# rlorenzo/facet

Measured on AMD Instinct MI355X. Metric: images/sec whole-node (TOPIQ+SAMP+CLIP+InsightFace ensemble), 1024² batch, higher is better.
Workload: dtype f32

## Files before the change

facet_amd/csrc/engine.hip:

```cpp
#include "engine.h"
#include "onnx_graph.h"
#include "wino64_maps.h"
#include <algorithm>
#include <cmath>
#include <cstdlib>

namespace fe {

void WeightStore::set(const std::string& name, const float* data, const int64_t* shape, int ndim) {
  HostTensor h;
  h.shape.assign(shape, shape + ndim);
  h.data.assign(data, data + h.numel());
  t_[name] = std::move(h);
}
const HostTensor& WeightStore::get(const std::string& name) const {
  auto it = t_.find(name);
  if (it == t_.end()) throw Error("missing weight tensor '" + name + "'");
  return it->second;
}

float* DeviceWeights::upload(const std::vector<float>& v) {
  void* p = nullptr;
  const size_t b = v.size() * sizeof(float);
  FE_HIP(hipMalloc(&p, b ? b : 16));
// ... 213 lines not shown

void conv_forward(Ctx& c, const ConvW& w, const Tensor& x, const Tensor& y, const ConvOpts& o) {
  FE_CHECK(x.c == w.CinPad, "conv: input channels %d != packed Cin %d", x.c, w.CinPad);
  FE_CHECK(y.c == w.Cout && y.n == x.n, "conv: output view mismatch (c=%d Cout=%d)", y.c, w.Cout);
  ConvParams p{};
  p.x = x.p; p.ldx = x.ld;
  p.w = w.w; p.scale = w.scale; p.shift = w.shift; p.slope = w.slope;
  FE_CHECK(o.act != ACT_PRELU || w.slope, "conv: PReLU without slopes");
  if (o.res) {
    FE_CHECK(o.res->c == y.c && o.res->pixels() == y.pixels(), "conv: residual shape mismatch");
    p.res = o.res->p; p.ldr = o.res->ld;
  }
  if (o.gate) {
    FE_CHECK(o.gate->pixels() == y.pixels() && (o.gate->c == 1 || o.gate->c == y.c), "conv: gate shape mismatch");
    p.gate = o.gate->p; p.ldg = o.gate->ld; p.gate_c1 = o.gate->c == 1;
  }
  p.y = y.p; p.ldy = y.ld;
  p.N = x.n; p.H = x.h; p.W = x.w; p.Cin = w.CinPad;
  p.Ho = y.h; p.Wo = y.w; p.Cout = w.Cout;
  p.KH = w.KH; p.KW = w.KW; p.sh = o.sh; p.sw = o.sw; p.ph = o.ph; p.pw = o.pw; p.dh = o.dh; p.dw = o.dw;
  FE_CHECK(y.h == conv_out_dim(x.h, w.KH, o.sh, o.ph, o.dh) && y.w == conv_out_dim(x.w, w.KW, o.sw, o.pw, o.dw),
           "conv: output dims %dx%d inconsistent with input %dx%d", y.h, y.w, x.h, x.w);
  p.K = w.K; p.Kp = w.Kp;
  p.M = (int)y.pixels();
  FE_CHECK(y.pixels() < (1ull << 31), "conv: M too large");
  p.act = o.act; p.res_after_act = o.res_after_act;
  p.variant = c.force_variant;
  if (w.wtap && o.act != ACT_PRELU && o.sh == 1 && o.sw == 1 && !o.res && !o.gate && p.variant == 0 && y.h == x.h && y.w == x.w) {
    const int T = w.KH * w.KW * w.Cout, Tp = (T + 3) & ~3;
    const size_t mark = c.arena.mark();
    Tensor z = c.arena.tensor(x.n, x.h, x.w, Tp);
    ConvParams q{};
    q.x = x.p; q.ldx = x.ld; q.w = w.wtap; q.y = z.p; q.ldy = Tp;
    q.N = x.n; q.H = x.h; q.W = x.w; q.Cin = w.CinPad; q.Ho = x.h; q.Wo = x.w; q.Cout = T;
    q.KH = q.KW = 1; q.sh = q.sw = q.dh = q.dw = 1;
    q.K = w.CinPad; q.Kp = w.KpT; q.M = (int)x.pixels();
    launch_conv(q, c.stream);
    launch_tap_gather(z.p, Tp, x.n, x.h, x.w, w.KH, w.KW, o.ph, o.pw, o.dh, o.dw, w.Cout, w.scale, w.shift, o.act, y.p,
                      y.ld, y.h, y.w, c.stream);
    c.arena.rewind(mark);
    c.flops_accum += 2.0 * p.M * (double)(w.KH * w.KW * w.Cin) * (w.CoutAlg ? w.CoutAlg : p.Cout);
    return;
  }
  static const bool no_wino = getenv("FE_NO_WINO") != nullptr;
  const bool wino_plain = !o.res && (o.act == ACT_NONE || o.act == ACT_RELU);
  if (w.wino && !no_wino && p.variant == 0 && o.sh == 1 && o.sw == 1 && o.ph == 1 && o.pw == 1 && o.dh == 1 && o.dw == 1 &&
      !o.gate && (wino_plain || (w.wino_m == 4 && (o.act == ACT_NONE || o.act == ACT_RELU || o.act == ACT_PRELU))) && y.h == x.h && y.w == x.w && (((uintptr_t)x.p | (uintptr_t)y.p) & 15) == 0 &&
      x.ld % 4 == 0 && y.ld % 4 == 0) {
    const int ts = w.wino_m, planes = (ts + 2) * (ts + 2);
    const int th = (x.h + ts - 1) / ts, tw = (x.w + ts - 1) / ts;
    const size_t tiles = (size_t)x.n * th * tw;
    const size_t wino_bytes = (size_t)planes * tiles * ((size_t)w.CinPad + w.Cout) * sizeof(float) + 1024;
    if (tiles < (1u << 30) / 36 && c.arena.mark() + wino_bytes <= c.arena.capacity()) {
      const size_t mark = c.arena.mark();
      float* V = (float*)c.arena.alloc((size_t)planes * tiles * w.CinPad * sizeof(float));
      float* Mb = (float*)c.arena.alloc((size_t)planes * tiles * w.Cout * sizeof(float));
      hipEvent_t e0 = nullptr, e1 = nullptr;
      if (c.profile) {
        FE_HIP(hipEventCreate(&e0)); FE_HIP(hipEventCreate(&e1));
        FE_HIP(hipEventRecord(e0, c.stream));
      }
      if (ts == 2) launch_wino_input(x, th, tw, V, c.stream);
      else launch_wino4_input(x, th, tw, V, c.stream);
      ConvParams g{};
      g.x = V; g.ldx = w.CinPad; g.w = w.wino; g.ldw = w.CinPad; g.y = Mb; g.ldy = w.Cout;
      g.M = (int)tiles; g.K = w.CinPad; g.Cout = w.Cout;
      g.N = 1; g.H = 1; g.W = g.M; g.Ho = 1; g.Wo = g.M; g.KH = g.KW = 1; g.sh = g.sw = g.dh = g.dw = 1;
      g.Kp = w.CinPad; g.Cin = w.CinPad;
      g.batch = planes; g.nb1 = 1; g.xs2 = (long long)tiles * w.CinPad; g.ws2 = (long long)w.Cout * w.CinPad; g.ys2 = (long long)tiles * w.Cout;
      launch_conv(g, c.stream);
      if (ts == 2) launch_wino_output(Mb, y, th, tw, w.scale, w.shift, o.act == ACT_RELU, c.stream);
      else launch_wino4_output(Mb, y, th, tw, w.scale, w.shift, o.act, w.slope, o.res, o.res_after_act, c.stream);
      if (c.profile) {
        FE_HIP(hipEventRecord(e1, c.stream));
        FE_HIP(hipEventSynchronize(e1));
        float ms = 0.f;
        FE_HIP(hipEventElapsedTime(&ms, e0, e1));
        (void)hipEventDestroy(e0); (void)hipEventDestroy(e1);
        char nm[128];
        snprintf(nm, sizeof nm, "wino3x3 M=%d K=%d N=%d", p.M, p.K, p.Cout);
        c.timings.push_back({nm, 2.0 * p.M * (double)(9 * w.Cin) * p.Cout, 0.0, ms});
      }
      c.arena.rewind(mark);
      c.flops_accum += 2.0 * p.M * (double)(w.KH * w.KW * w.Cin) * (w.CoutAlg ? w.CoutAlg : p.Cout);
      c.flops_saved += 2.0 * p.M * (double)(9 * w.Cin) * (w.CoutAlg ? w.CoutAlg : p.Cout) - 2.0 * (double)planes * (double)tiles * w.CinPad * w.Cout;
      return;
    }
  }
  static const bool no_wino64 = getenv("FE_NO_WINO64") != nullptr;
  if (w.wino64 && !no_wino64 && p.variant == 0 && (o.act == ACT_NONE || o.act == ACT_RELU || o.act == ACT_PRELU) && o.sh == 1 && o.sw == 1 && o.ph == 1 && o.pw == 1 && o.dh == 1 && o.dw == 1 && !o.gate && y.h == x.h &&
      y.w == x.w && (((uintptr_t)x.p | (uintptr_t)y.p | (uintptr_t)(o.res ? o.res->p : nullptr)) & 15) == 0 && x.ld % 4 == 0 && y.ld % 4 == 0 &&
      (!o.res || o.res->ld % 4 == 0) && (unsigned long long)x.h * x.w * x.ld * 4ull < 0xF0000000ull) {
    hipEvent_t e0 = nullptr, e1 = nullptr;
    if (c.profile) {
      FE_HIP(hipEventCreate(&e0)); FE_HIP(hipEventCreate(&e1));
      FE_HIP(hipEventRecord(e0, c.stream));
    }
    launch_wino64(x, y, w.wino64, w.scale, w.shift, w.slope, o.act, o.res, o.res_after_act, c.stream);
    const double direct = 2.0 * p.M * (double)(9 * w.Cin) * (w.CoutAlg ? w.CoutAlg : p.Cout);
    if (c.profile) {
      FE_HIP(hipEventRecord(e1, c.stream));
      FE_HIP(hipEventSynchronize(e1));
      float ms = 0.f;
      FE_HIP(hipEventElapsedTime(&ms, e0, e1));
      (void)hipEventDestroy(e0); (void)hipEventDestroy(e1);
      char nm[128];
      snprintf(nm, sizeof nm, "wino64 3x3 M=%d K=%d N=%d", p.M, p.K, p.Cout);
      const double bytes = 4.0 * ((double)x.pixels() * x.c + (double)y.pixels() * y.c * (o.res ? 2 : 1) + (double)w64::U_FLOATS);
      c.timings.push_back({nm, direct, bytes, ms});
    }
    const double tiles = (double)x.n * ((x.h + 1) / 2) * ((x.w + 1) / 2);
    c.flops_accum += direct;
    c.flops_saved += direct - 2.0 * 16.0 * tiles * 64.0 * w.Cout;
    return;
  }
  static const bool no_splitk = getenv("FE_NO_SPLITK") != nullptr;
  static const int splitk_min = getenv("FE_SPLITK_MIN") ? atoi(getenv("FE_SPLITK_MIN")) : 2048;
  if (!no_splitk && w.KH == 1 && w.KW == 1 && o.sh == 1 && o.sw == 1 && o.ph == 0 && o.pw == 0 && !o.gate && p.variant == 0 && p.M <= 256 &&
      w.CinPad >= splitk_min && w.K == w.CinPad && (size_t)((p.M + 127) / 128) * ((w.Cout + 63) / 64) < 64 &&
      (o.act == ACT_NONE || o.act == ACT_RELU || o.act == ACT_PRELU)) {
    int splits = 0;
    for (int s = 64; s >= 2; --s)
      if (w.CinPad % s == 0 && (w.CinPad / s) % 32 == 0 && w.CinPad / s >= 256) { splits = s; break; }
    const size_t part_bytes = (size_t)splits * p.M * w.Cout * sizeof(float);
    if (splits && c.arena.mark() + part_bytes + 1024 <= c.arena.capacity()) {
      const size_t mark = c.arena.mark();
      float* part = (float*)c.arena.alloc(part_bytes);
      const int Ks = w.CinPad / splits;
      hipEvent_t e0 = nullptr, e1 = nullptr;
      if (c.profile) {
        FE_HIP(hipEventCreate(&e0)); FE_HIP(hipEventCreate(&e1));
        FE_HIP(hipEventRecord(e0, c.stream));
      }
      ConvParams g{};
      g.x = x.p; g.ldx = x.ld; g.w = w.w; g.ldw = w.Kp; g.y = part; g.ldy = w.Cout;
      g.M = p.M; g.K = Ks; g.Kp = Ks; g.Cin = Ks; g.Cout = w.Cout;
      g.N = 1; g.H = 1; g.W = g.M; g.Ho = 1; g.Wo = g.M; g.KH = g.KW = 1; g.sh = g.sw = g.dh = g.dw = 1;
      g.batch = splits; g.nb1 = 1; g.xs2 = Ks; g.ws2 = Ks; g.ys2 = (long long)p.M * w.Cout;
      launch_conv(g, c.stream);
      launch_splitk_reduce(part, splits, p.M, w.Cout, w.scale, w.shift, w.slope, o.act, o.res ? o.res->p : nullptr, o.res ? o.res->ld : 0,
                           o.res_after_act, y.p, y.ld, c.stream);
      if (c.profile) {
        FE_HIP(hipEventRecord(e1, c.stream));
        FE_HIP(hipEventSynchronize(e1));
        float ms = 0.f;
        FE_HIP(hipEventElapsedTime(&ms, e0, e1));
        (void)hipEventDestroy(e0); (void)hipEventDestroy(e1);
        char nm[128];
        snprintf(nm, sizeof nm, "splitk%d 1x1 M=%d K=%d N=%d", splits, p.M, p.K, p.Cout);
        c.timings.push_back({nm, 2.0 * p.M * (double)w.Cin * (w.CoutAlg ? w.CoutAlg : p.Cout), 0.0, ms});
      }
      c.arena.rewind(mark);
      c.flops_accum += 2.0 * p.M * (double)w.Cin * (w.CoutAlg ? w.CoutAlg : p.Cout);
      return;
    }
  }
  static const bool no_stem = getenv("FE_NO_STEM") != nullptr;
  const bool stem = w.wstem && !no_stem && p.variant == 0 && o.sh == o.sw && o.ph == w.KH / 2 && o.pw == w.KW / 2 && o.dh == 1 && o.dw == 1 && !o.res &&
                    !o.gate && (o.act == ACT_NONE || o.act == ACT_RELU || o.act == ACT_PRELU);
  auto launch = [&]() {
    if (stem && launch_stem(x.p, x.ld, x.n, x.h, x.w, w.wstem, w.scale, w.shift, w.slope, w.Cout, w.KH, o.sh,
                            o.act == ACT_RELU ? 1 : (o.act == ACT_PRELU ? 2 : 0), y.p, y.ld, y.h, y.w, c.stream))
      return;
    launch_conv(p, c.stream);
  };
  if (c.profile) {
    hipEvent_t e0, e1;
    FE_HIP(hipEventCreate(&e0)); FE_HIP(hipEventCreate(&e1));
    FE_HIP(hipEventRecord(e0, c.stream));
    launch();
    FE_HIP(hipEventRecord(e1, c.stream));
    FE_HIP(hipEventSynchronize(e1));
    float ms = 0.f;
    FE_HIP(hipEventElapsedTime(&ms, e0, e1));
    (void)hipEventDestroy(e0); (void)hipEventDestroy(e1);
    char nm[128];
    snprintf(nm, sizeof nm, "conv%dx%d s%d d%d M=%d K=%d N=%d", w.KH, w.KW, o.sh, o.dh, p.M, p.K, p.Cout);
    double bytes = 4.0 * ((double)x.pixels() * x.c + (double)y.pixels() * y.c * (o.res ? 2 : 1) + (double)w.Cout * w.K);
    c.timings.push_back({nm, 2.0 * p.M * (double)(w.KH * w.KW * w.Cin) * (w.CoutAlg ? w.CoutAlg : p.Cout), bytes, ms});
  } else {
    launch();
  }
  c.flops_accum += 2.0 * p.M * (double)(w.KH * w.KW * w.Cin) * (w.CoutAlg ? w.CoutAlg : p.Cout);
}

template <class E>
static void conv_forward_half(Ctx& c, const ConvW& w, const TensorT<E>& x, const TensorT<E>& y, const ConvOptsT<E>& o) {
  if (!w.wh && w.w && PrecOf<E>::value != PREC_F32 && !o.res && !o.gate && x.ld == x.c && y.ld == y.c && x.c >= w.CinPad) {
    const size_t mark = c.arena.mark();
    Tensor xf = c.arena.tensor(x.n, x.h, x.w, x.c), yf = c.arena.tensor(y.n, y.h, y.w, y.c);
    launch_convert(x.p, xf.p, x.numel(), c.stream);
    ConvOpts of; of.sh = o.sh; of.sw = o.sw; of.ph = o.ph; of.pw = o.pw; of.dh = o.dh; of.dw = o.dw; of.act = o.act;
    conv_forward(c, w, xf.slice(0, w.CinPad), yf, of);
    launch_convert(yf.p, y.p, y.numel(), c.stream);
    c.arena.rewind(mark);
    return;
  }
  FE_CHECK(w.wh && w.hprec == PrecOf<E>::value, "conv(2-byte): this layer has no weights of the activations' type (model committed under another "
           "precision, or a 3-channel first layer)");
  FE_CHECK(x.c == w.CinPadH, "conv(bf16): input channels %d != packed Cin %d", x.c, w.CinPadH);
  FE_CHECK(y.c == w.Cout && y.n == x.n, "conv(bf16): output view mismatch (c=%d Cout=%d)", y.c, w.Cout);
  FE_CHECK(y.p || o.y32, "conv(2-byte): no output tensor");
  FE_CHECK(y.h == conv_out_dim(x.h, w.KH, o.sh, o.ph, o.dh) && y.w == conv_out_dim(x.w, w.KW, o.sw, o.pw, o.dw),
           "conv(bf16): output dims %dx%d inconsistent with input %dx%d", y.h, y.w, x.h, x.w);
  FE_CHECK(y.pixels() < (1ull << 31), "conv: M too large");
  const double flops = 2.0 * (double)y.pixels() * (double)(w.KH * w.KW * w.Cin) * (w.CoutAlg ? w.CoutAlg : w.Cout);
  hipEvent_t e0 = nullptr, e1 = nullptr;
  if (c.profile) {
    FE_HIP(hipEventCreate(&e0)); FE_HIP(hipEventCreate(&e1));
    FE_HIP(hipEventRecord(e0, c.stream));
  }
  ConvParamsT<E> p{};
  p.scale = w.scale; p.shift = w.shift; p.slope = w.slope;
  p.N = x.n; p.H = x.h; p.W = x.w; p.Cin = w.CinPadH; p.x = x.p; p.ldx = x.ld;
  if (w.wtap_h && o.act != ACT_PRELU && o.sh == 1 && o.sw == 1 && !o.res && !o.gate && !o.res32 && !o.y32 && y.h == x.h && y.w == x.w) {
    const int T = w.KH * w.KW * w.Cout, T8 = (T + 7) & ~7;
    const size_t mark = c.arena.mark();
    TensorT<E> z = c.arena.tensor_t<E>(x.n, x.h, x.w, T8);
    p.w = (const E*)w.wtap_h; p.y = z.p; p.ldy = T8; p.scale = p.shift = p.slope = nullptr;
    p.Ho = x.h; p.Wo = x.w; p.Cout = T8; p.KH = p.KW = 1; p.sh = p.sw = p.dh = p.dw = 1;
    p.K = w.CinPadH; p.Kp = w.KpTH; p.M = (int)x.pixels(); p.cb = 32;
    launch_conv_bf16(p, c.stream);
    launch_tap_gather(z.p, T8, x.n, x.h, x.w, w.KH, w.KW, o.ph, o.pw, o.dh, o.dw, w.Cout, w.scale, w.shift, o.act, y.p, y.ld, y.h, y.w, c.stream);
    c.arena.rewind(mark);
  } else {
    FE_CHECK(o.act != ACT_PRELU || w.slope, "conv: PReLU without slopes");
    if (o.res) {
      FE_CHECK(o.res->c == y.c && o.res->pixels() == y.pixels(), "conv: residual shape mismatch");
      p.res = o.res->p; p.ldr = o.res->ld;
    }
    if (o.gate) {
      FE_CHECK(o.gate->pixels() == y.pixels() && (o.gate->c == 1 || o.gate->c == y.c), "conv: gate shape mismatch");
      p.gate = o.gate->p; p.ldg = o.gate->ld; p.gate_c1 = o.gate->c == 1;
    }
    if (o.res32) {
      FE_CHECK(!o.res && o.res32->c == y.c && o.res32->pixels() == y.pixels(), "conv: fp32 residual shape mismatch");
      p.res32 = o.res32->p; p.ldr32 = o.res32->ld;
    }
    if (o.y32) {
      FE_CHECK(o.y32->c == y.c && o.y32->pixels() == y.pixels(), "conv: fp32 output shape mismatch");
      p.y32 = o.y32->p; p.ldy32 = o.y32->ld;
    }
    p.w = (const E*)w.wh; p.y = y.p; p.ldy = y.ld;
    p.Ho = y.h; p.Wo = y.w; p.Cout = w.Cout;
    p.KH = w.KH; p.KW = w.KW; p.sh = o.sh; p.sw = o.sw; p.ph = o.ph; p.pw = o.pw; p.dh = o.dh; p.dw = o.dw;
    p.K = w.KH * w.KW * w.CinPadH; p.Kp = w.KpH; p.M = (int)y.pixels(); p.cb = w.cb;
    p.act = o.act; p.res_after_act = o.res_after_act;
    p.variant = c.force_variant;
    launch_conv_bf16(p, c.stream);
  }
  if (c.profile) {
    FE_HIP(hipEventRecord(e1, c.stream));
    FE_HIP(hipEventSynchronize(e1));
    float ms = 0.f;
    FE_HIP(hipEventElapsedTime(&ms, e0, e1));
    (void)hipEventDestroy(e0); (void)hipEventDestroy(e1);
    char nm[128];
    snprintf(nm, sizeof nm, "%s conv%dx%d s%d d%d M=%d K=%d N=%d", PrecOf<E>::value == PREC_F16 ? "f16" : "bf16", w.KH, w.KW, o.sh, o.dh, (int)y.pixels(), w.KH * w.KW * w.Cin, w.Cout);
    const double bytes = 2.0 * ((double)x.pixels() * x.c + (double)y.pixels() * y.c * (o.res ? 2 : 1) + (double)w.Cout * w.KpH);
    c.timings.push_back({nm, flops, bytes, ms});
  }
  c.flops_accum += flops;
  c.flops_half += flops;
}
void conv_forward(Ctx& c, const ConvW& w, const TensorH& x, const TensorH& y, const ConvOptsT<bf16>& o) { conv_forward_half<bf16>(c, w, x, y, o); }
void conv_forward(Ctx& c, const ConvW& w, const TensorF16& x, const TensorF16& y, const ConvOptsT<f16>& o) { conv_forward_half<f16>(c, w, x, y, o); }

template <class T>
TensorT<T> conv_new(Ctx& c, const ConvW& w, const TensorT<T>& x, const ConvOptsT<T>& o) {
  TensorT<T> y = c.arena.tensor_t<T>(x.n, conv_out_dim(x.h, w.KH, o.sh, o.ph, o.dh), conv_out_dim(x.w, w.KW, o.sw, o.pw, o.dw), w.Cout);
  conv_forward(c, w, x, y, o);
  return y;
}
template Tensor conv_new<float>(Ctx&, const ConvW&, const Tensor&, const ConvOpts&);
template TensorH conv_new<bf16>(Ctx&, const ConvW&, const TensorH&, const ConvOptsT<bf16>&);
template TensorF16 conv_new<f16>(Ctx&, const ConvW&, const TensorF16&, const ConvOptsT<f16>&);

template <>
Tensor first_conv<float>(Ctx& c, const ConvW& w, const Tensor& x, const ConvOpts& o) { return conv_new(c, w, x, o); }
template <class E>
static TensorT<E> first_conv_half(Ctx& c, const ConvW& w, const Tensor& x, const ConvOpts& o) {
  const int ho = conv_out_dim(x.h, w.KH, o.sh, o.ph, o.dh), wo = conv_out_dim(x.w, w.KW, o.sw, o.pw, o.dw);
  TensorT<E> y = c.arena.tensor_t<E>(x.n, ho, wo, w.Cout);
  static const bool no_stem = getenv("FE_NO_STEM") != nullptr;
  const bool stem = w.wstem && !no_stem && o.sh == o.sw && o.ph == w.KH / 2 && o.pw == w.KW / 2 && o.dh == 1 && o.dw == 1 && !o.res && !o.gate &&
                    (o.act == ACT_NONE || o.act == ACT_RELU || o.act == ACT_PRELU);
  if (stem && launch_stem(x.p, x.ld, x.n, x.h, x.w, w.wstem, w.scale, w.shift, w.slope, w.Cout, w.KH, o.sh,
                          o.act == ACT_RELU ? 1 : (o.act == ACT_PRELU ? 2 : 0), y.p, y.ld, ho, wo, c.stream)) {
    c.flops_accum += 2.0 * (double)y.pixels() * (double)(w.KH * w.KW * w.Cin) * w.Cout;
    if (w.KH == 7) c.flops_half += 2.0 * (double)y.pixels() * (double)(w.KH * w.KW * w.Cin) * w.Cout;
    return y;
  }
  const size_t mark = c.arena.mark();
  Tensor yf = conv_new(c, w, x, o);
  launch_convert(yf.p, y.p, y.numel(), c.stream);
  (void)mark;
  return y;
}
template <>
TensorH first_conv<bf16>(Ctx& c, const ConvW& w, const Tensor& x, const ConvOpts& o) { return first_conv_half<bf16>(c, w, x, o); }
template <>
TensorF16 first_conv<f16>(Ctx& c, const ConvW& w, const Tensor& x, const ConvOpts& o) { return first_conv_half<f16>(c, w, x, o); }

void build_resnet(ResNet& r, DeviceWeights& dw, const WeightStore& ws, const std::string& prefix,
                  bool bottleneck, const int blocks[4], bool seq_names) {
  r.bottleneck = bottleneck;
// ... 344 lines not shown
```

facet_amd/csrc/fe_common.h:

```cpp
#pragma once
#include <hip/hip_runtime.h>
#include "fe_check.h"
#include <cstdint>
#include <cstdio>
#include <atomic>
#include <cstring>
#include <map>
#include <mutex>
#include <stdexcept>
#include <string>
#include <vector>

namespace fe {


#define FE_HIP(expr)                                                                      \
  do {                                                                                    \
    hipError_t _e = (expr);                                                               \
    if (_e != hipSuccess) {                                                               \
      char _b[512];                                                                       \
      snprintf(_b, sizeof _b, "%s:%d: %s -> %s", __FILE__, __LINE__, #expr,               \
               hipGetErrorString(_e));                                                    \
      throw fe::Error(_b);                                                                \
    }                                                                                     \
// ... 107 lines not shown
using TensorH = TensorT<bf16>;
using TensorF16 = TensorT<f16>;

__device__ __forceinline__ float ldf(const float* p) { return *p; }
__device__ __forceinline__ float ldf(const bf16* p) { return (float)*p; }
__device__ __forceinline__ void stf(float* p, float v) { *p = v; }
__device__ __forceinline__ void stf(bf16* p, float v) { *p = (bf16)v; }
__device__ __forceinline__ float ldf(const f16* p) { return (float)*p; }
__device__ __forceinline__ void stf(f16* p, float v) { *p = fe_to_f16(v); }
__device__ __forceinline__ float4 ld4(const float* p) { return *reinterpret_cast<const float4*>(p); }
__device__ __forceinline__ float4 ld4(const bf16* p) {
  const uint2 u = *reinterpret_cast<const uint2*>(p);
  return make_float4(__uint_as_float(u.x << 16), __uint_as_float(u.x & 0xFFFF0000u), __uint_as_float(u.y << 16), __uint_as_float(u.y & 0xFFFF0000u));
}
__device__ __forceinline__ float4 ld4(const f16* p) {
  const uint2 u = *reinterpret_cast<const uint2*>(p);
  float4 v;
  fe_unpack2(p, u.x, v.x, v.y); fe_unpack2(p, u.y, v.z, v.w);
  return v;
}
__device__ __forceinline__ void st4(float* p, float4 v) { *reinterpret_cast<float4*>(p) = v; }
__device__ __forceinline__ void st4(f16* p, float4 v) {
  *reinterpret_cast<uint2*>(p) = make_uint2(fe_pack2(p, v.x, v.y), fe_pack2(p, v.z, v.w));
}
__device__ __forceinline__ void st4(bf16* p, float4 v) {
  typedef __bf16 bf4 __attribute__((ext_vector_type(4)));
  bf4 o; o[0] = (bf16)v.x; o[1] = (bf16)v.y; o[2] = (bf16)v.z; o[3] = (bf16)v.w;
  *reinterpret_cast<bf4*>(p) = o;
}

class Arena {
 public:
  void init(size_t bytes) {
    release();
    FE_HIP(hipMalloc(&base_, bytes));
    cap_ = bytes;
    off_ = 0;
  }
  void release() {
    if (base_) (void)hipFree(base_);
    base_ = nullptr;
    cap_ = off_ = 0;
  }
  ~Arena() { release(); }
  void reset() { off_ = 0; }
  size_t mark() const { return off_; }
  void rewind(size_t m) { off_ = m; }
  size_t capacity() const { return cap_; }
  size_t high_water() const { return high_; }
  void* alloc(size_t bytes) {
    size_t a = (off_ + 255) & ~(size_t)255;
    FE_CHECK(a + bytes <= cap_, "arena exhausted: need %zu at %zu of %zu", bytes, a, cap_);
    off_ = a + bytes;
    if (off_ > high_) high_ = off_;
    return (char*)base_ + a;
  }
  template <class T>
  TensorT<T> tensor_t(int n, int h, int w, int c) {
    TensorT<T> t;
    t.n = n; t.h = h; t.w = w; t.c = c; t.ld = c;
    t.p = (T*)alloc(t.numel() * sizeof(T));
    return t;
  }
  Tensor tensor(int n, int h, int w, int c) { return tensor_t<float>(n, h, w, c); }
  template <class T>
  T* array(size_t count) { return (T*)alloc(count * sizeof(T)); }
 private:
  void* base_ = nullptr;
  size_t cap_ = 0, off_ = 0, high_ = 0;
};

template <class T>
struct ConvParamsT {
  const T* x; int ldx;
  const T* w;
  const float* scale;
  const float* shift;
  const float* slope;
  const T* res; int ldr;
  const T* gate; int ldg;
  T* y; int ldy;
  int N, H, W, Cin, Ho, Wo, Cout;
  int KH, KW, sh, sw, ph, pw, dh, dw;
  int K, Kp, M;
  int act;
  int res_after_act;
  int gate_c1;
  int vec_epi;
  int unit_stride;
  int ldw;
  int batch, nb1;
  long long xs1, xs2, ws1, ws2, ys1, ys2, hs1;
  int buf_ok; unsigned x_span, w_span;
  unsigned y_span, r_span, g_span;
  int variant;
  int cb;
  int pad_store;
  const float* res32; int ldr32;
  float* y32; int ldy32;
  unsigned r32_span, y32_span;
  int a_wrap;
  int split_lo_off;
  int exact_act;
};
using ConvParams = ConvParamsT<float>;
using ConvParamsH = ConvParamsT<bf16>;

struct ConvW {
  float* w = nullptr;
  float* scale = nullptr;
  float* shift = nullptr;
  float* slope = nullptr;
  int Cout = 0, Cin = 0, CinPad = 0, KH = 1, KW = 1, K = 0, Kp = 0;
  int CoutAlg = 0;
  float* wtap = nullptr;
  int wino_m = 0;
  float* wino = nullptr;
  float* wino64 = nullptr;
  float* wstem = nullptr;
  float* wn16 = nullptr;
  int KpT = 0;
  void* wh = nullptr;
  int hprec = 0;
  int KpH = 0, cb = 0, CinPadH = 0;
  void* wtap_h = nullptr;
  int KpTH = 0;
  uint8_t* w8 = nullptr;
  float* w8_scale = nullptr;
};

template <class T>
struct ConvOptsT {
  int sh = 1, sw = 1, ph = 0, pw = 0, dh = 1, dw = 1;
  int act = ACT_NONE;
  const TensorT<T>* res = nullptr;
  int res_after_act = 0;
  const TensorT<T>* gate = nullptr;
  const TensorT<float>* res32 = nullptr;
  const TensorT<float>* y32 = nullptr;
};
using ConvOpts = ConvOptsT<float>;

constexpr int CONV_KALIGN = 32;
constexpr int CONV_KALIGN_H = 64;

void launch_conv(const ConvParams& p, hipStream_t s);
void launch_wino_input(const Tensor& x, int th, int tw, float* V, hipStream_t s);
void launch_wino_output(const float* Mb, const Tensor& y, int th, int tw, const float* scale, const float* shift, int relu, hipStream_t s);
void launch_wino4_input(const Tensor& x, int th, int tw, float* V, hipStream_t s);
void launch_wino4_output(const float* Mb, const Tensor& y, int th, int tw, const float* scale, const float* shift, int act, const float* slope,
                         const Tensor* res, int res_after_act, hipStream_t s);
void launch_wino64(const Tensor& x, const Tensor& y, const float* U, const float* scale, const float* shift, const float* slope, int act,
                   const Tensor* res, int res_after_act, hipStream_t s);
template <class TO>
bool launch_stem(const float* x, int ldx, int N, int H, int W, const float* wstem, const float* scale, const float* shift, const float* slope,
                 int Cout, int k, int stride, int act, TO* y, int ldy, int Ho, int Wo, hipStream_t s);
void launch_conv_narrow(const ConvParams& p, hipStream_t s);
void launch_conv_dma(const ConvParams& p, int tile, hipStream_t s);
void launch_conv_bf16(const ConvParamsH& p, hipStream_t s);
void launch_conv_bf16(const ConvParamsT<f16>& p, hipStream_t s);
template <class T, class Launch>
inline bool conv_split_by_images(const ConvParamsT<T>& p, Launch&& launch) {
  if (p.batch > 1 || p.N <= 1 || (long long)p.N * p.Ho * p.Wo != (long long)p.M) return false;
  const unsigned long long in_img = (unsigned long long)p.H * p.W * p.ldx * sizeof(T);
  unsigned long long out_img = (unsigned long long)p.Ho * p.Wo * (unsigned long long)(p.ldy > p.ldr ? p.ldy : p.ldr) * sizeof(T);
  const unsigned long long out32_img = (unsigned long long)p.Ho * p.Wo * (unsigned long long)(p.ldy32 > p.ldr32 ? p.ldy32 : p.ldr32) * sizeof(float);
  if ((p.y32 || p.res32) && out32_img > out_img) out_img = out32_img;
  const unsigned long long per_img = in_img > out_img ? in_img : out_img;
  constexpr unsigned long long LIMIT = 0xF0000000ull;
  if (per_img >= LIMIT) return false;
  const int ng = (int)(LIMIT / per_img);
  if (ng >= p.N) return false;
  for (int i0 = 0; i0 < p.N; i0 += ng) {
    ConvParamsT<T> q = p;
    const int n = ng < p.N - i0 ? ng : p.N - i0;
    const size_t opix = (size_t)i0 * p.Ho * p.Wo;
    q.N = n; q.M = n * p.Ho * p.Wo;
    q.x = p.x + (size_t)i0 * p.H * p.W * p.ldx;
    if (p.y) q.y = p.y + opix * p.ldy;
    if (p.y32) q.y32 = p.y32 + opix * p.ldy32;
    if (p.res32) q.res32 = p.res32 + opix * p.ldr32;
    if (p.res) q.res = p.res + opix * p.ldr;
    if (p.gate) q.gate = p.gate + opix * p.ldg;
    launch(q);
  }
  return true;
}

double conv_flops(const ConvParams& p);

void launch_u8_to_nhwc4_norm(const uint8_t* src, float* dst, size_t pixels, const float mean[3],
                             const float stdv[3], int bgr, hipStream_t s);
template <class T> void launch_nchw_to_nhwc(const float* src, T* dst, int n, int c, int h, int w, int cpad, hipStream_t s);
template <class T> void launch_nhwc_to_nchw(const T* src, int lds_, float* dst, int n, int c, int h, int w, hipStream_t s);
template <class T> void launch_maxpool(const TensorT<T>& x, const TensorT<T>& y, int k, int stride, int pad, hipStream_t s);
template <class T> void launch_bilinear(const TensorT<T>& x, const TensorT<T>& y, hipStream_t s);
template <class T> void launch_adaptive_avgpool(const TensorT<T>& x, const TensorT<T>& y, hipStream_t s);
void launch_convert(const float* x, bf16* y, size_t n, hipStream_t s);
void launch_convert(const bf16* x, float* y, size_t n, hipStream_t s);
void launch_convert(const float* x, f16* y, size_t n, hipStream_t s);
void launch_convert(const f16* x, float* y, size_t n, hipStream_t s);
void launch_splitk_reduce(const float* part, int splits, int M, int N, const float* scale, const float* shift, const float* slope, int act,
                          const float* res, int ldr, int res_after_act, float* y, int ldy, hipStream_t s);
template <class T>
void launch_tap_gather(const T* z, int ldz, int n, int h, int w, int kh, int kw, int ph, int pw, int dh, int dw,
                       int cout, const float* scale, const float* shift, int act, T* y, int ldy, int ho, int wo,
                       hipStream_t s);
void launch_attention(const float* q, int ldq, const float* k, int ldk, const float* vt, int lp, const float* bv, float* o,
                      int ldo, int B, int H, int Lq, int Lk, int dmodel, int causal, hipStream_t s);
void launch_attention(const bf16* q, int ldq, const bf16* k, int ldk, const bf16* vt, int lp, const float* bv, bf16* o,
                      int ldo, int B, int H, int Lq, int Lk, int dmodel, int causal, hipStream_t s);
void launch_attention(const f16* q, int ldq, const f16* k, int ldk, const f16* vt, int lp, const float* bv, f16* o,
                      int ldo, int B, int H, int Lq, int Lk, int dmodel, int causal, hipStream_t s);
void launch_attention_split(const f16* q, const f16* k, int ld, int lo_off, const f16* vt_hi, const f16* vt_lo, int lp, f16* o, int ldo, int o_lo_off,
                            int B, int H, int Lq, int Lk, int dmodel, hipStream_t s);
template <class TI, class TW, class TO>
void launch_gemm_skinny(const TI* x, int ldx, const TW* w, int ldw, const float* scale, const float* shift, TO* y,
                        int ldy, int M, int N, int K, int act, hipStream_t s);
void launch_sigmoid(const Tensor& x, const Tensor& y, hipStream_t s);
void launch_add(const Tensor& a, const Tensor& b, const Tensor& y, hipStream_t s);
void launch_layernorm_split(const float* x, int ldx, f16* y, int ldy, const float* g, const float* b, int rows, int d, float eps, hipStream_t s);
void launch_split_hi_lo(const float* x, f16* y, size_t rows, int cols, hipStream_t s);
template <class T, class TO>
void launch_layernorm(const T* x, int ldx, TO* y, int ldy, const float* g, const float* b,
                      int rows, int d, float eps, hipStream_t s);
void launch_softmax_rows(float* x, int ld, int rows, int d, hipStream_t s);
void launch_softmax_rows_pad(float* x, int ld, int rows, int d, hipStream_t s);
template <class T>
void launch_add_rows_bcast(T* y, int ldy, const float* pos, int rows, int L, int d, hipStream_t s);

void launch_affine_act(const Tensor& x, const Tensor& y, const float* scale, const float* shift, int act, const float* slope,
                       hipStream_t s);
void launch_binary(const Tensor& a, const Tensor& b, const Tensor& y, int op, int act, hipStream_t s);
void launch_gather_strided(const float* src, float* dst, const long long dims[6], const long long sstr[6], hipStream_t s);
void launch_nearest(const Tensor& x, const Tensor& y, hipStream_t s);
void launch_avgpool(const Tensor& x, const Tensor& y, int k, int stride, int pad, int include_pad, hipStream_t s);
void launch_dwconv(const Tensor& x, const Tensor& y, const float* wt, int kh, int kw, int sh, int sw, int ph, int pw,
                   const float* scale, const float* shift, int act, const float* slope, const Tensor* res, hipStream_t s);

void launch_cv_resize_linear(const uint8_t* src, int n, int h, int w, uint8_t* dst, int ch, int cw, int nh, int nw, const int* xofs,
                             const short* ialpha, const int* yofs, const short* ibeta, int area2, hipStream_t s);
void launch_warp_affine(const uint8_t* src, int h, int w, const int* img_of, const double* Minv, int m, int S, const short* wtab,
                        uint8_t* dst, hipStream_t s);
void launch_swap_rb_u8(const uint8_t* src, uint8_t* dst, size_t pixels, hipStream_t s);
void launch_u8_blob(const uint8_t* src, float* dst, size_t pixels, float mean, float scale, int swap_rb, hipStream_t s);
void launch_scrfd_decode(const float* scores, const float* bbox, const float* kps, int n, int fh, int fw, int A, int K, int stride,
                         float thresh, float det_scale, int level, float* cand, int* counts, int max_cand, hipStream_t s);
void cv_resize_tables(int src, int dst, bool clamp_fx, std::vector<int>& ofs, std::vector<short>& coef);
void cv_warp_weight_table(std::vector<short>& wtab);

constexpr int FE_STATS_COUNT = 264;
size_t stats_accum_bytes(int n);
void launch_image_stats(const uint8_t* bgr, int n, int h, int w, uint8_t* gray, uint8_t* hsv_out, const int* sdiv, const int* hdiv, void* accum,
                        double* out, hipStream_t s);
void cv_hsv_tables(std::vector<int>& sdiv, std::vector<int>& hdiv);
void launch_roi_laplacian(const uint8_t* bgr, int h, int w, const int* img_of, const int* rois, int m, double* out, hipStream_t s);
void launch_canny_map(const uint8_t* d_bgr, int n, int h, int w, int low, int high, uint8_t* d_blur, void* d_grad, void* d_mag, uint8_t* d_map,
                      hipStream_t s);
void launch_canny_map_gray(const uint8_t* d_gray, int n, int h, int w, const int* d_thr, void* d_grad, void* d_mag, uint8_t* d_map, hipStream_t s);
struct ContourScratch {
  int* lab_fg;
  int* lab_bg;
  int* cnt;
  int* strong;
  int* xmin;
  int* xmax;
  int* ymax;
  uint8_t* outer;
  uint8_t* edge;
  int* work;
  int* work_count;
  long long* recs;
  int* rec_count;
  int* error;
};
constexpr int FE_CONTOUR_RECORD = 8;
int contour_work_cap(int h, int w);
size_t contour_scratch_bytes(int nb, int h, int w);
void contour_scratch_carve(ContourScratch& sc, void* base, int nb, int h, int w);
void launch_median_thresholds(const double* d_stats, int n, long long npx, int* d_thr, hipStream_t s);
void launch_external_contours(const uint8_t* d_img, int nb, int h, int w, int candidates, long long min_twice_area, ContourScratch& sc,
                              hipStream_t s);

}
```

Before: 237.8.

## Add persistent streaming MFMA kernel for small-K 1x1 convolutions

Adds a dedicated kernel for unpadded stride-1 1x1 convolutions with K in {64,128,256}. It keeps weights resident in registers and streams input rows into LDS through double-buffered buffer-to-LDS loads, with a persistent grid sized to resident blocks. The epilogue (scale/shift, activation, residual, gate) is fused and staged through LDS for coalesced float4 stores. This targets the memory-bound behaviour of the generic conv path on these layers, at the cost of narrow shape and alignment conditions and fragile hand-written asm waitcnt scheduling.

```diff
diff --git a/facet_amd/csrc/engine.hip b/facet_amd/csrc/engine.hip
--- a/facet_amd/csrc/engine.hip
+++ b/facet_amd/csrc/engine.hip
@@ -389,6 +389,38 @@
       }
       c.arena.rewind(mark);
       c.flops_accum += 2.0 * p.M * (double)w.Cin * (w.CoutAlg ? w.CoutAlg : p.Cout);
+      return;
+    }
+  }
+  static const bool no_stream1x1 = getenv("FE_NO_STREAM1X1") != nullptr;
+  {
+    auto al16 = [](const void* ptr) { return ((uintptr_t)ptr & 15) == 0; };
+    const unsigned long long xspan = ((unsigned long long)x.pixels() - 1) * (unsigned long long)x.ld * 4 + (unsigned long long)w.CinPad * 4;
+    if (!no_stream1x1 && p.variant == 0 && w.KH == 1 && w.KW == 1 && o.sh == 1 && o.sw == 1 && o.ph == 0 && o.pw == 0 && o.dh == 1 && o.dw == 1 &&
+        y.h == x.h && y.w == x.w && w.K == w.CinPad && w.Kp == w.CinPad && stream1x1_supports(w.CinPad, w.Cout) && w.Cout % 4 == 0 &&
+        (o.act == ACT_NONE || o.act == ACT_RELU || o.act == ACT_GELU || o.act == ACT_SIGMOID) && !(o.res && o.gate && o.gate->c != 1) &&
+        al16(x.p) && al16(w.w) && al16(y.p) && x.ld % 4 == 0 && y.ld % 4 == 0 && (!o.res || (al16(o.res->p) && o.res->ld % 4 == 0)) &&
+        (!o.gate || o.gate->c == 1 || (al16(o.gate->p) && o.gate->ld % 4 == 0)) && (!w.scale || al16(w.scale)) && (!w.shift || al16(w.shift)) &&
+        xspan < 0xFFFFFF00ull) {
+      hipEvent_t e0 = nullptr, e1 = nullptr;
+      if (c.profile) {
+        FE_HIP(hipEventCreate(&e0)); FE_HIP(hipEventCreate(&e1));
+        FE_HIP(hipEventRecord(e0, c.stream));
+      }
+      launch_stream1x1(p, c.stream);
+      const double flops = 2.0 * p.M * (double)w.Cin * (w.CoutAlg ? w.CoutAlg : p.Cout);
+      if (c.profile) {
+        FE_HIP(hipEventRecord(e1, c.stream));
+        FE_HIP(hipEventSynchronize(e1));
+        float ms = 0.f;
+        FE_HIP(hipEventElapsedTime(&ms, e0, e1));
+        (void)hipEventDestroy(e0); (void)hipEventDestroy(e1);
+        char nm[128];
+        snprintf(nm, sizeof nm, "stream1x1 M=%d K=%d N=%d", p.M, p.K, p.Cout);
+        const double bytes = 4.0 * ((double)x.pixels() * x.c + (double)y.pixels() * y.c * (o.res ? 2 : 1) + (double)w.Cout * w.K);
+        c.timings.push_back({nm, flops, bytes, ms});
+      }
+      c.flops_accum += flops;
       return;
     }
   }
diff --git a/facet_amd/csrc/fe_common.h b/facet_amd/csrc/fe_common.h
--- a/facet_amd/csrc/fe_common.h
+++ b/facet_amd/csrc/fe_common.h
@@ -283,6 +283,8 @@
                          const Tensor* res, int res_after_act, hipStream_t s);
 void launch_wino64(const Tensor& x, const Tensor& y, const float* U, const float* scale, const float* shift, const float* slope, int act,
                    const Tensor* res, int res_after_act, hipStream_t s);
+bool stream1x1_supports(int K, int N);
+void launch_stream1x1(const ConvParams& p, hipStream_t s);
 template <class TO>
 bool launch_stem(const float* x, int ldx, int N, int H, int W, const float* wstem, const float* scale, const float* shift, const float* slope,
                  int Cout, int k, int stride, int act, TO* y, int ldy, int Ho, int Wo, hipStream_t s);
diff --git a/facet_amd/csrc/kernels_stream1x1.hip b/facet_amd/csrc/kernels_stream1x1.hip
--- /dev/null
+++ b/facet_amd/csrc/kernels_stream1x1.hip
@@ -0,0 +1,264 @@
+#include "fe_common.h"
+#include "stream1x1_maps.h"
+
+namespace fe {
+
+typedef __attribute__((address_space(3))) void* s1_lptr_t;
+
+template <int K, int BM, int WM, int WN, int TM, int TN>
+__global__ __launch_bounds__(256, (TM * TN == 1 ? (K <= 64 ? 4 : (K <= 128 ? 3 : 2)) : 2)) void stream1x1_kernel(const ConvParams p, const int ntiles) {
+  using namespace s1x1;
+  constexpr int NKC = K / KC, CW = TN * 32, PN = WN * CW;
+  constexpr int SLAB_FLOATS = slab_floats(BM), STEP_FLOATS = step_floats(BM), PIECES_PER_WAVE = pieces_per_wave(BM);
+  constexpr int ES = CW + 4, LPR = CW / 4, RPI = 64 / LPR, NIT = 32 / RPI, NAUX = TM * NIT;
+  static_assert(WM * WN == 4 && WM * TM * 32 == BM, "4 waves over the tile");
+  extern __shared__ __attribute__((aligned(16))) float smem[];
+
+  const int t0 = tile_begin(blockIdx.x, gridDim.x, ntiles), t1 = tile_begin(blockIdx.x + 1, gridDim.x, ntiles);
+  if (t0 >= t1) return;
+  const int n0 = blockIdx.y * PN;
+
+  const int t = threadIdx.x, lane = t & 63, wave = __builtin_amdgcn_readfirstlane(t >> 6);
+  const int wm = wave / WN, wn = wave % WN;
+  const int r = lane & 31, h = lane >> 5;
+
+  fe_v4f bf[NKC][TN][SLABS][2];
+#pragma unroll
+  for (int kc = 0; kc < NKC; ++kc)
+#pragma unroll
+    for (int j = 0; j < TN; ++j)
+#pragma unroll
+      for (int sl = 0; sl < SLABS; ++sl)
+#pragma unroll
+        for (int s = 0; s < 2; ++s)
+          bf[kc][j][sl][s] = *reinterpret_cast<const fe_v4f*>(p.w + (size_t)(n0 + wn * CW + j * 32 + r) * p.ldw + kc * KC + k_of(sl, s, h, 0));
+
+  const __amdgpu_buffer_rsrc_t rsA = __builtin_amdgcn_make_buffer_rsrc(const_cast<float*>(p.x), 0, (int)p.x_span, 0x00020000);
+  const int prow = piece_row(BM, wave, lane), pchunk = piece_src_chunk(lane) * 4;
+  char* const sbytes = reinterpret_cast<char*>(smem);
+  auto issue_step = [&](const int step, const int buf) __attribute__((always_inline)) {
+    const int tile = t0 + step / NKC, kc = step % NKC;
+    int m = tile * BM + prow;
+    m = m < p.M ? m : p.M - 1;
+    const unsigned off = (unsigned)(((long long)m * p.ldx + pchunk) * 4);
+#pragma unroll
+    for (int j = 0; j < PIECES_PER_WAVE; ++j)
+      __builtin_amdgcn_raw_ptr_buffer_load_lds(rsA, (s1_lptr_t)(sbytes + buf * (STEP_FLOATS * 4) + piece_dst_float(BM, wave, j, 0) * 4), 16, (int)off,
+                                               (kc * KC + piece_slab(BM, wave, j) * 16) * 4, 0, 0);
+  };
+
+  const int lr = epi_row(CW, lane, 0), lc = epi_col(CW, lane);
+  const int colb = n0 + wn * CW + lc;
+  float4 sc = make_float4(1.f, 1.f, 1.f, 1.f), sf = make_float4(0.f, 0.f, 0.f, 0.f);
+  if (p.scale) sc = *reinterpret_cast<const float4*>(p.scale + colb);
+  if (p.shift) sf = *reinterpret_cast<const float4*>(p.shift + colb);
+  const bool has_res = p.res != nullptr, gate_c1 = p.gate && p.gate_c1, gate_full = p.gate && !p.gate_c1;
+  const bool has_aux = has_res || gate_full;
+  const float* const auxp = has_res ? p.res : p.gate;
+  const int ldaux = has_res ? p.ldr : p.ldg;
+  const int act = p.act;
+
+  const unsigned lds_base = (unsigned)(size_t)(s1_lptr_t)smem;
+  const unsigned e_base = lds_base + 2u * STEP_FLOATS * 4u + (unsigned)wave * (32u * ES * 4u);
+  const unsigned e_wr = e_base + (unsigned)epi_write_float(CW, 0, h, r) * 4u;
+  const unsigned e_rd = e_base + (unsigned)(lr * ES + lc) * 4u;
+  const unsigned a_rd0 = lds_base + (unsigned)frag_float(BM, 0, wm * TM * 32 + r, 0, h) * 4u;
+  const unsigned a_rd1 = lds_base + (unsigned)frag_float(BM, 0, wm * TM * 32 + r, 1, h) * 4u;
+
+#pragma unroll
+  for (int kc = 0; kc < NKC; ++kc)
+#pragma unroll
+    for (int j = 0; j < TN; ++j)
+#pragma unroll
+      for (int sl = 0; sl < SLABS; ++sl)
+#pragma unroll
+        for (int s = 0; s < 2; ++s) asm volatile("" : "+v"(bf[kc][j][sl][s]));
+  asm volatile("" : "+v"(sc.x), "+v"(sc.y), "+v"(sc.z), "+v"(sc.w), "+v"(sf.x), "+v"(sf.y), "+v"(sf.z), "+v"(sf.w));
+
+  fe_v4f auxn[NAUX];
+  float gsn[NAUX];
+  auto request_aux = [&](const int tile) __attribute__((always_inline)) {
+    const int mrow = tile * BM + wm * TM * 32 + lr;
+    if (has_aux) {
+#pragma unroll
+      for (int a = 0; a < NAUX; ++a) {
+        const int m = mrow + (a / NIT) * 32 + (a % NIT) * RPI;
+        auxn[a] = *reinterpret_cast<const fe_v4f*>(auxp + (size_t)(m < p.M ? m : p.M - 1) * ldaux + colb);
+      }
+    }
+    if (gate_c1) {
+#pragma unroll
+      for (int a = 0; a < NAUX; ++a) {
+        const int m = mrow + (a / NIT) * 32 + (a % NIT) * RPI;
+        gsn[a] = p.gate[(size_t)(m < p.M ? m : p.M - 1) * p.ldg];
+      }
+    }
+  };
+
+  const int nsteps = (t1 - t0) * NKC;
+  issue_step(0, 0);
+  if (nsteps > 1) {
+    issue_step(1, 1);
+    asm volatile("s_waitcnt vmcnt(%0)" ::"i"(PIECES_PER_WAVE) : "memory");
+  } else {
+    asm volatile("s_waitcnt vmcnt(0)" ::: "memory");
+  }
+  __builtin_amdgcn_s_barrier();
+
+  int step = 0;
+  unsigned cur = 0;
+  for (int tile = t0; tile < t1; ++tile) {
+    fe_f32x16 acc[TM][TN];
+#pragma unroll
+    for (int i = 0; i < TM; ++i)
+#pragma unroll
+      for (int j = 0; j < TN; ++j)
+#pragma unroll
+        for (int e = 0; e < 16; ++e) acc[i][j][e] = 0.f;
+    fe_v4f aux[NAUX];
+    float gs[NAUX];
+    const int mrow0 = tile * BM + wm * TM * 32 + lr;
+
+#pragma unroll
+    for (int kc = 0; kc < NKC; ++kc) {
+      if (kc == NKC - 1) request_aux(tile);
+      fe_v4f fa[2][2 * TM];
+#define S1_READ(SET, SL)                                                                                                              \
+  _Pragma("unroll") for (int i = 0; i < TM; ++i) {                                                                                    \
+    asm volatile("ds_read_b128 %0, %1 offset:%2" : "=v"(fa[SET][2 * i]) : "v"(a_rd0 + cur), "i"(((SL) * SLAB_FLOATS + i * 512) * 4));     \
+    asm volatile("ds_read_b128 %0, %1 offset:%2" : "=v"(fa[SET][2 * i + 1]) : "v"(a_rd1 + cur), "i"(((SL) * SLAB_FLOATS + i * 512) * 4)); \
+  }
+      S1_READ(0, 0)
+      asm volatile("s_waitcnt lgkmcnt(0)" ::: "memory");
+      __builtin_amdgcn_sched_barrier(0);
+#pragma unroll
+      for (int sl = 0; sl < SLABS; ++sl) {
+        if (sl + 1 < SLABS) {
+          if (sl & 1) { S1_READ(0, sl + 1) } else { S1_READ(1, sl + 1) }
+        }
+        __builtin_amdgcn_sched_barrier(0);
+#pragma unroll
+        for (int s = 0; s < 2; ++s)
+#pragma unroll
+          for (int i = 0; i < TM; ++i)
+#pragma unroll
+            for (int j = 0; j < TN; ++j) {
+              const fe_v4f a = fa[sl & 1][2 * i + s], b = bf[kc][j][sl][s];
+              acc[i][j] = __builtin_amdgcn_mfma_f32_32x32x2f32(a.x, b.x, acc[i][j], 0, 0, 0);
+              acc[i][j] = __builtin_amdgcn_mfma_f32_32x32x2f32(a.y, b.y, acc[i][j], 0, 0, 0);
+              acc[i][j] = __builtin_amdgcn_mfma_f32_32x32x2f32(a.z, b.z, acc[i][j], 0, 0, 0);
+              acc[i][j] = __builtin_amdgcn_mfma_f32_32x32x2f32(a.w, b.w, acc[i][j], 0, 0, 0);
+            }
+        asm volatile("s_waitcnt lgkmcnt(0)" : "+v"(acc[TM - 1][TN - 1])::"memory");
+        __builtin_amdgcn_sched_barrier(0);
+      }
+#undef S1_READ
+      asm volatile("s_waitcnt vmcnt(0)" ::: "memory");
+      __builtin_amdgcn_s_barrier();
+      if (kc == NKC - 1) {
+#pragma unroll
+        for (int a = 0; a < NAUX; ++a) {
+          asm volatile("" : "+v"(auxn[a]), "+v"(gsn[a]));
+          aux[a] = auxn[a]; gs[a] = gsn[a];
+        }
+      }
+      __builtin_amdgcn_sched_barrier(0);
+      if (step + 2 < nsteps) issue_step(step + 2, (int)(cur != 0));
+      __builtin_amdgcn_sched_barrier(0);
+      ++step;
+      cur ^= (unsigned)(STEP_FLOATS * 4);
+    }
+
+    asm volatile("s_nop 15\n\ts_nop 15" ::: "memory");
+#pragma unroll
+    for (int i = 0; i < TM; ++i) {
+#pragma unroll
+      for (int j = 0; j < TN; ++j)
+#pragma unroll
+        for (int e = 0; e < 16; ++e)
+          asm volatile("ds_write_b32 %0, %1 offset:%2" ::"v"(e_wr), "v"(acc[i][j][e]), "i"((acc_row(e, 0) * ES + j * 32) * 4) : "memory");
+      asm volatile("s_waitcnt lgkmcnt(0)" ::: "memory");
+      fe_v4f ev[NIT];
+#pragma unroll
+      for (int it = 0; it < NIT; ++it) asm volatile("ds_read_b128 %0, %1 offset:%2" : "=v"(ev[it]) : "v"(e_rd), "i"(it * RPI * ES * 4) : "memory");
+      asm volatile("s_waitcnt lgkmcnt(0)" ::: "memory");
+      __builtin_amdgcn_sched_barrier(0);
+#pragma unroll
+      for (int it = 0; it < NIT; ++it) {
+        const int m = mrow0 + i * 32 + it * RPI;
+        const fe_v4f rv = aux[i * NIT + it];
+        float4 v = make_float4(ev[it].x * sc.x + sf.x, ev[it].y * sc.y + sf.y, ev[it].z * sc.z + sf.z, ev[it].w * sc.w + sf.w);
+        if (has_res && !p.res_after_act) { v.x += rv.x; v.y += rv.y; v.z += rv.z; v.w += rv.w; }
+        if (act == ACT_RELU) {
+          v.x = fe_apply_act(v.x, ACT_RELU); v.y = fe_apply_act(v.y, ACT_RELU); v.z = fe_apply_act(v.z, ACT_RELU); v.w = fe_apply_act(v.w, ACT_RELU);
+        } else if (act == ACT_GELU) {
+          v.x = fe_apply_act(v.x, ACT_GELU); v.y = fe_apply_act(v.y, ACT_GELU); v.z = fe_apply_act(v.z, ACT_GELU); v.w = fe_apply_act(v.w, ACT_GELU);
+        } else if (act == ACT_SIGMOID) {
+          v.x = fe_apply_act(v.x, ACT_SIGMOID); v.y = fe_apply_act(v.y, ACT_SIGMOID); v.z = fe_apply_act(v.z, ACT_SIGMOID); v.w = fe_apply_act(v.w, ACT_SIGMOID);
+        }
+        if (has_res && p.res_after_act) { v.x += rv.x; v.y += rv.y; v.z += rv.z; v.w += rv.w; }
+        if (gate_full) { v.x *= rv.x; v.y *= rv.y; v.z *= rv.z; v.w *= rv.w; }
+        if (gate_c1) {
+          const float g = gs[i * NIT + it];
+          asm("v_mul_f32 %0, %0, %1" : "+v"(v.x) : "v"(g));
+          asm("v_mul_f32 %0, %0, %1" : "+v"(v.y) : "v"(g));
+          asm("v_mul_f32 %0, %0, %1" : "+v"(v.z) : "v"(g));
+          asm("v_mul_f32 %0, %0, %1" : "+v"(v.w) : "v"(g));
+        }
+        if (m < p.M) *reinterpret_cast<float4*>(p.y + (size_t)m * p.ldy + colb) = v;
+      }
+    }
+  }
+}
+
+template <int K, int BM, int WM, int WN, int TM, int TN>
+static void launch_stream1x1_form(const ConvParams& p, hipStream_t s) {
+  using namespace s1x1;
+  constexpr int PN = WN * TN * 32;
+  constexpr size_t lds = (size_t)2 * step_floats(BM) * 4 + (size_t)4 * 32 * (TN * 32 + 4) * 4;
+  auto kern = stream1x1_kernel<K, BM, WM, WN, TM, TN>;
+  static std::atomic<uint64_t> lds_set{0};
+  ensure_dynamic_lds((const void*)kern, lds, lds_set);
+  static const int resident = [&]() {
+    int dev = 0, cus = 0, per = 0;
+    FE_HIP(hipGetDevice(&dev));
+    FE_HIP(hipDeviceGetAttribute(&cus, hipDeviceAttributeMultiprocessorCount, dev));
+    FE_HIP(hipOccupancyMaxActiveBlocksPerMultiprocessor(&per, kern, 256, lds));
+    const int by_lds = (int)((160u * 1024u) / lds);
+    per = per < 1 ? 1 : (per > by_lds ? by_lds : per);
+    return cus * (per > 4 ? 4 : per);
+  }();
+  const int ntiles = (p.M + BM - 1) / BM, panels = p.Cout / PN;
+  int grid = resident / panels;
+  grid = grid < 1 ? 1 : (grid > ntiles ? ntiles : grid);
+  hipLaunchKernelGGL(kern, dim3(grid, panels), dim3(256), lds, s, p, ntiles);
+  FE_HIP(hipGetLastError());
+}
+
+bool stream1x1_supports(int K, int N) {
+  s1x1::Form f;
+  return s1x1::form_of(K, N, f);
+}
+
+void launch_stream1x1(const ConvParams& p0, hipStream_t s) {
+  FE_CHECK(p0.KH == 1 && p0.KW == 1 && p0.sh == 1 && p0.sw == 1 && p0.ph == 0 && p0.pw == 0 && p0.batch <= 1 && p0.K == p0.Cin && p0.Kp == p0.Cin,
+           "stream1x1: 1x1, stride 1, unpadded, unbatched layers only");
+  FE_CHECK(stream1x1_supports(p0.Cin, p0.Cout), "stream1x1: %d -> %d is outside the family", p0.Cin, p0.Cout);
+  FE_CHECK(p0.act == ACT_NONE || p0.act == ACT_RELU || p0.act == ACT_GELU || p0.act == ACT_SIGMOID, "stream1x1: activation %d", p0.act);
+  FE_CHECK(!(p0.res && p0.gate && !p0.gate_c1), "stream1x1: a residual and a full gate together");
+  ConvParams p = p0;
+  if (p.ldw == 0) p.ldw = p.Kp;
+  auto al16 = [](const void* ptr) { return ((uintptr_t)ptr & 15) == 0; };
+  FE_CHECK(al16(p.x) && al16(p.w) && al16(p.y) && p.ldx % 4 == 0 && p.ldw % 4 == 0 && p.ldy % 4 == 0 && (!p.res || (al16(p.res) && p.ldr % 4 == 0)) &&
+               (!p.gate || p.gate_c1 || (al16(p.gate) && p.ldg % 4 == 0)) && (!p.scale || al16(p.scale)) && (!p.shift || al16(p.shift)),
+           "stream1x1: operands must be 16-byte aligned");
+  const unsigned long long xs = ((unsigned long long)p.M - 1) * (unsigned long long)p.ldx * 4 + (unsigned long long)p.Cin * 4;
+  FE_CHECK(xs < 0xFFFFFF00ull, "stream1x1: the input spans more than 32-bit buffer offsets address");
+  p.x_span = (unsigned)xs;
+  if (p.Cin == 64 && p.Cout == 64) launch_stream1x1_form<64, 64, 2, 2, 1, 1>(p, s);
+  else if (p.Cin == 256 && p.Cout == 64) launch_stream1x1_form<256, 64, 2, 2, 1, 1>(p, s);
+  else if (p.Cin == 64 && p.Cout == 256) launch_stream1x1_form<64, 32, 1, 4, 1, 2>(p, s);
+  else launch_stream1x1_form<128, 32, 1, 4, 1, 1>(p, s);
+}
+
+}
diff --git a/facet_amd/csrc/stream1x1_maps.h b/facet_amd/csrc/stream1x1_maps.h
--- /dev/null
+++ b/facet_amd/csrc/stream1x1_maps.h
@@ -0,0 +1,46 @@
+#pragma once
+
+#if defined(__HIPCC__)
+#define S1_HD __host__ __device__ __forceinline__
+#else
+#define S1_HD inline
+#endif
+
+namespace fe {
+namespace s1x1 {
+
+constexpr int KC = 64;
+constexpr int SLABS = KC / 16;
+S1_HD constexpr int slab_floats(int BM) { return BM * 16; }
+S1_HD constexpr int step_floats(int BM) { return BM * KC; }
+S1_HD constexpr int pieces_per_wave(int BM) { return BM / 16; }
+
+S1_HD int tile_begin(int b, int G, int T) { return (int)((long long)b * T / G); }
+
+S1_HD int piece_slab(int BM, int wave, int j) { return (wave / (BM / 16)) * pieces_per_wave(BM) + j; }
+S1_HD int piece_row(int BM, int wave, int lane) { return 16 * (wave % (BM / 16)) + (lane >> 2); }
+S1_HD int piece_src_chunk(int lane) { return (lane & 3) ^ (((lane >> 2) >> 2) & 3); }
+S1_HD int piece_dst_float(int BM, int wave, int j, int lane) { return piece_slab(BM, wave, j) * slab_floats(BM) + 256 * (wave % (BM / 16)) + 4 * lane; }
+
+S1_HD int frag_float(int BM, int slab, int row, int s, int h) { return slab * slab_floats(BM) + row * 16 + (((2 * s + h) ^ ((row >> 2) & 3)) << 2); }
+S1_HD int k_of(int slab, int s, int h, int e) { return 16 * slab + 8 * s + 4 * h + e; }
+S1_HD int acc_row(int e, int h) { return (e & 3) + 8 * (e >> 2) + 4 * h; }
+
+S1_HD int epi_stride(int CW) { return CW + 4; }
+S1_HD int epi_write_float(int CW, int e, int h, int col) { return acc_row(e, h) * epi_stride(CW) + col; }
+S1_HD int epi_lanes_per_row(int CW) { return CW / 4; }
+S1_HD int epi_rows_per_iter(int CW) { return 64 / epi_lanes_per_row(CW); }
+S1_HD int epi_iters(int CW) { return 32 / epi_rows_per_iter(CW); }
+S1_HD int epi_row(int CW, int lane, int it) { return lane / epi_lanes_per_row(CW) + it * epi_rows_per_iter(CW); }
+S1_HD int epi_col(int CW, int lane) { return (lane % epi_lanes_per_row(CW)) * 4; }
+
+struct Form { int BM, WM, WN, TM, TN; };
+S1_HD bool form_of(int K, int N, Form& f) {
+  if ((K == 64 || K == 256) && N == 64) { f = Form{64, 2, 2, 1, 1}; return true; }
+  if (K == 64 && N == 256) { f = Form{32, 1, 4, 1, 2}; return true; }
+  if (K == 128 && N >= 128 && N % 128 == 0) { f = Form{32, 1, 4, 1, 1}; return true; }
+  return false;
+}
+
+}
+}
```

Result: no change. 240.1 (median of 6 runs) (+0.9%).
